# CogitatorTech/vq

Hardware: AMD Instinct MI355X
Metric: pq_encode_vectors_per_s (higher is better)
Workload: dtype f32 (bf16x3-split MFMA screen, exact f32 re-check)

## Files before the change

include/vqhip.h:

```cpp
#ifndef VQHIP_H
#define VQHIP_H

#include <stddef.h>
#include <stdint.h>

#ifdef __cplusplus
extern "C" {
#endif

#define VQHIP_VERSION_MAJOR 0
#define VQHIP_VERSION_MINOR 1

#define VQHIP_OK 0
#define VQHIP_ERR_NULL_PTR (-1)
#define VQHIP_ERR_INVALID_INPUT (-3)
#define VQHIP_ERR_NO_DEVICE (-4)
#define VQHIP_ERR_RUNTIME (-5)
#define VQHIP_ERR_UNSUPPORTED (-6)
#define VQHIP_ERR_FAILURE (-99)

#define VQHIP_SQUARED_EUCLIDEAN 0
#define VQHIP_EUCLIDEAN 1
#define VQHIP_MANHATTAN 2
#define VQHIP_COSINE 3
// ... 13 lines not shown
const char *vqhip_backend(void);
const char *vqhip_last_error(void);
int vqhip_device_count(void);
int vqhip_set_device(int device);
int vqhip_get_device(int *device);
int vqhip_set_stream(void *hip_stream);
int vqhip_synchronize(void);
int vqhip_selftest(float *bf16_32x32x16_ratio, float *bf16_16x16x32_ratio, int *bf16_engine_trusted);
int vqhip_mfma_bf16_probe(const uint16_t *a, const uint16_t *b, const float *c, uint64_t trials, float *d);
int vqhip_mfma_bf16_model(const uint16_t *a, const uint16_t *b, const float *c, uint64_t trials, float *d);
int vqhip_mfma_bf16_model_check(uint64_t trials, uint64_t seed, uint64_t *mismatches, uint64_t *first_bad_trial);
int vqhip_mfma_bf16_model_failures(uint64_t trials, uint64_t seed, uint64_t *trial_ids, uint32_t cap, uint64_t *n_failures);
int vqhip_mfma_bf16_model_case(uint64_t seed, uint64_t trial, uint16_t *a, uint16_t *b, float *c);
int vqhip_last_assign_stats(uint64_t *rechecked, int *engine);
int vqhip_last_screen_products(int *products);

int vqhip_set_profiling(int on);
int vqhip_profile_collect(uint32_t *n_calls, double *primary_ms, double *recheck_ms);
int vqhip_xfer_lane_calls(uint64_t *calls);
int vqhip_memcpy_device(void *dst, const void *src, uint64_t bytes);

int vqhip_dataset_from_host(const float *rows, uint64_t n, uint32_t d, vqhip_dataset **out);
int vqhip_dataset_from_device(const void *dev_rows, uint64_t n, uint32_t d, vqhip_dataset **out);
int vqhip_dataset_synthetic(uint64_t n, uint32_t d, uint64_t seed, uint64_t row_offset,
                            vqhip_dataset **out);
int vqhip_dataset_info(const vqhip_dataset *ds, uint64_t *n, uint32_t *d, const void **dev_rows);
int vqhip_dataset_read(const vqhip_dataset *ds, uint64_t row0, uint64_t nrows, float *out);
int vqhip_dataset_destroy(vqhip_dataset *ds);
int vqhip_synth_uniform_host(float *out, uint64_t n, uint32_t d, uint64_t seed,
                             uint64_t row_offset);
// ... 283 lines not shown
```

vq_amd/_lib.py:

```python
from __future__ import annotations

import ctypes as C
import os

import numpy as np

from . import _arena

from .errors import FfiError

_HERE = os.path.dirname(os.path.abspath(__file__))
LIB_PATH = os.environ.get("VQHIP_LIB_PATH", os.path.join(_HERE, "libvqhip.so"))

OK = 0
ERR_NULL_PTR, ERR_INVALID_INPUT, ERR_NO_DEVICE, ERR_RUNTIME, ERR_UNSUPPORTED, ERR_FAILURE = (
    -1, -3, -4, -5, -6, -99)

SQUARED_EUCLIDEAN, EUCLIDEAN, MANHATTAN, COSINE, COSINE_UNCLAMPED = 0, 1, 2, 3, 4
IVF_RESIDUAL = 1
ENGINE_AUTO, ENGINE_EXACT, ENGINE_MFMA, ENGINE_MFMA_BF16 = 0, 1, 2, 3

_u8p = C.POINTER(C.c_uint8)
_u16p = C.POINTER(C.c_uint16)
_u32p = C.POINTER(C.c_uint32)
# ... 1 lines not shown
_i32p = C.POINTER(C.c_int32)
_f32p = C.POINTER(C.c_float)
_vp = C.c_void_p
_vpp = C.POINTER(C.c_void_p)

SIGNATURES = {
    "vqhip_backend": (C.c_char_p, []),
    "vqhip_last_error": (C.c_char_p, []),
    "vqhip_device_count": (C.c_int, []),
    "vqhip_set_device": (C.c_int, [C.c_int]),
    "vqhip_get_device": (C.c_int, [C.POINTER(C.c_int)]),
    "vqhip_set_stream": (C.c_int, [_vp]),
    "vqhip_synchronize": (C.c_int, []),
    "vqhip_last_assign_stats": (C.c_int, [_u64p, C.POINTER(C.c_int)]),
    "vqhip_last_screen_products": (C.c_int, [C.POINTER(C.c_int)]),
    "vqhip_xfer_lane_calls": (C.c_int, [C.POINTER(C.c_uint64)]),
    "vqhip_set_profiling": (C.c_int, [C.c_int]),
    "vqhip_profile_collect": (C.c_int, [_u32p, C.POINTER(C.c_double), C.POINTER(C.c_double)]),
    "vqhip_memcpy_device": (C.c_int, [_vp, _vp, C.c_uint64]),
    "vqhip_code_bytes": (C.c_uint32, [C.c_uint32]),
    "vqhip_dataset_from_host": (C.c_int, [_f32p, C.c_uint64, C.c_uint32, _vpp]),
    "vqhip_dataset_from_device": (C.c_int, [_vp, C.c_uint64, C.c_uint32, _vpp]),
    "vqhip_dataset_synthetic": (C.c_int, [C.c_uint64, C.c_uint32, C.c_uint64, C.c_uint64, _vpp]),
    "vqhip_dataset_info": (C.c_int, [_vp, _u64p, _u32p, _vpp]),
    "vqhip_dataset_read": (C.c_int, [_vp, C.c_uint64, C.c_uint64, _f32p]),
    "vqhip_dataset_destroy": (C.c_int, [_vp]),
    "vqhip_synth_uniform_host": (C.c_int, [_f32p, C.c_uint64, C.c_uint32, C.c_uint64, C.c_uint64]),
    "vqhip_kmeans_create": (C.c_int, [_vp, C.c_uint32, C.c_uint32, _vpp]),
    "vqhip_kmeans_destroy": (C.c_int, [_vp]),
    "vqhip_kmeans_set_centroids": (C.c_int, [_vp, _f32p]),
# ... 1132 lines not shown
    check(load().vqhip_memcpy_device(C.c_void_p(dst), C.c_void_p(src), nbytes))


def last_assign_stats():
    r, e = C.c_uint64(), C.c_int()
    check(load().vqhip_last_assign_stats(C.byref(r), C.byref(e)))
    return int(r.value), int(e.value)


def last_screen_products() -> int:
    p = C.c_int()
    check(load().vqhip_last_screen_products(C.byref(p)))
    return int(p.value)


def param_check(rc: int) -> None:
    if rc == OK:
        return
    import re

    from .errors import InvalidParameter

    msg = last_error()
    m = re.fullmatch(r"Invalid parameter '([^']*)': (.*)", msg, flags=re.S)
    if rc == ERR_INVALID_INPUT and m:
        raise InvalidParameter(m.group(1), m.group(2))
    raise FfiError(msg or f"libvqhip status {rc}", rc)


def elementwise(fn: str, params, a, in_dtype, out_dtype, out=None) -> np.ndarray:
# ... 12 lines not shown
```

vq_amd/csrc/api.hip:

```cpp
#include <algorithm>
#include <atomic>
#include <cmath>
#include <cstdlib>
#include <cstring>
#include <limits>
#include <map>
#include <memory>
#include <condition_variable>
#include <mutex>
#include <new>
#include <thread>
#include <vector>

#include "adc_plan.hpp"
#include "kernels.hpp"

namespace vqhip {

ThreadState &tls() {
    static thread_local ThreadState st;
    return st;
}

int fail(int code, const char *fmt, ...) {
// ... 1020 lines not shown

int vqhip_mfma_bf16_model_case(uint64_t seed, uint64_t trial, uint16_t *a, uint16_t *b, float *c) {
    if (!a || !b || !c) return fail(VQHIP_ERR_NULL_PTR, "NULL argument");
    mfma_bf16_model_case(seed, trial, a, b, c);
    return VQHIP_OK;
}

int vqhip_synchronize(void) {
    VQ_TRY(require_gfx950());
    hipStream_t s;
    VQ_TRY(current_stream(&s));
    VQ_HIP(hipStreamSynchronize(s));
    return VQHIP_OK;
}

int vqhip_last_assign_stats(uint64_t *rechecked, int *engine) {
    VQ_API_BEGIN
    ThreadState &st = tls();
    if (engine) *engine = st.last_engine;
    if (rechecked) {
        *rechecked = 0;
        if (!g_last_ws) return VQHIP_OK;
        WsPin pin(g_last_ws);
        if (!pin.ws) return VQHIP_OK;
        AssignWorkspace *ws = pin.ws;
        Entry in(*pin.sync);
        if (ws->stats_pending) {
            hipStream_t s;
            VQ_TRY(in.stream(&s));
            uint64_t tot = 0;
            if (ws->last_segmented) {
                if (ws->last_n_seg > 0) {
                    VQ_HIP(hipMemcpyAsync(ws->seg_host, ws->wl_seg.p, (size_t)ws->stats_m * ws->last_n_seg * 8, hipMemcpyDeviceToHost, s));
                    VQ_HIP(hipStreamSynchronize(s));
                    for (size_t i = 0; i < (size_t)ws->stats_m * ws->last_n_seg; ++i) tot += ws->seg_host[2 * i + 1];
                }
            } else {
                VQ_HIP(hipMemcpyAsync(ws->stats_host, ws->wl_count.p, (size_t)ws->stats_m * 4, hipMemcpyDeviceToHost, s));
                VQ_HIP(hipStreamSynchronize(s));
                for (uint32_t i = 0; i < ws->stats_m; ++i) tot += ws->stats_host[i];
            }
            in.synced();
            *rechecked = tot;
        }
    }
    return VQHIP_OK;
    VQ_API_END
}

int vqhip_last_screen_products(int *products) {
    if (!products) return fail(VQHIP_ERR_NULL_PTR, "NULL argument");
    const ThreadState &st = tls();
    *products = (st.last_engine == VQHIP_ENGINE_MFMA_BF16) ? st.last_products : 0;
    return VQHIP_OK;
}

int vqhip_xfer_lane_calls(uint64_t *calls) {
    if (!calls) return fail(VQHIP_ERR_NULL_PTR, "NULL argument");
    *calls = g_xfer_lane_calls.load();
    return VQHIP_OK;
// ... 3166 lines not shown
```

vq_amd/csrc/k_exact.hip:

```cpp
#include "kernels.hpp"
#include <type_traits>

#pragma clang fp contract(off)

namespace vqhip {
namespace {

constexpr int kExactBlock = 256;

template <int METRIC, int SD, bool GENERIC>
__device__ __forceinline__ uint32_t scan_one(const float *__restrict__ xrow, uint32_t sd_rt,
                                             const float *__restrict__ cbs,
                                             const float *__restrict__ cnsq, uint32_t k) {
    const uint32_t sd = GENERIC ? sd_rt : (uint32_t)SD;
    float x[GENERIC ? 1 : SD];
    if constexpr (!GENERIC) {
#pragma unroll
        for (int t = 0; t < SD; ++t) x[t] = xrow[t];
    }
    float na = 0.0f;
    if constexpr (vq_is_cos(METRIC)) {
        float sa = -0.0f;
        if constexpr (GENERIC) {
            for (uint32_t t = 0; t < sd; ++t) {
// ... 203 lines not shown
                const float dist = acc[jj][r];
                if (j == 0) {
                    best_dist = dist;
                } else if (dist < best_dist) {
                    best_dist = dist;
                    best = j;
                }
            }
        }
        __syncthreads();
    }
    if (q == 0 && row0 + r < n) store_code(codes, (row0 + r) * m + s, best, k);
}

template <int METRIC, int SD>
__device__ __forceinline__ float exact_dist_fixed(const float (&x)[SD], const float *__restrict__ c,
                                                  float na, float nb) {
    if constexpr (METRIC == VQHIP_SQUARED_EUCLIDEAN || METRIC == VQHIP_EUCLIDEAN) {
        float acc = 0.0f;
#pragma unroll
        for (int t = 0; t < SD; ++t) {
            float diff = x[t] - c[t];
            float sq = diff * diff;
            acc = acc + sq;
        }
        return (METRIC == VQHIP_EUCLIDEAN) ? sqrtf(acc) : acc;
    } else if constexpr (METRIC == VQHIP_MANHATTAN) {
        float acc = 0.0f;
#pragma unroll
        for (int t = 0; t < SD; ++t) {
            float diff = x[t] - c[t];
            acc = acc + fabsf(diff);
        }
        return acc;
    } else {
        float dot = -0.0f;
#pragma unroll
        for (int t = 0; t < SD; ++t) {
            float p = x[t] * c[t];
            dot = dot + p;
        }
        return vq_cosine_finish(METRIC, dot, na, nb);
    }
}

template <int METRIC, int SD>
__global__ __launch_bounds__(1024) void k_recheck_wave(
    const float *__restrict__ X, uint32_t d, uint32_t m, uint32_t k,
    const float *__restrict__ cb, const float *__restrict__ cnsqrt,
    const uint32_t *__restrict__ sub_list, const uint32_t *__restrict__ wl_rows,
    const uint32_t *__restrict__ wl_count, uint64_t wl_stride, const uint32_t *__restrict__ wl_seg,
    uint32_t n_seg, uint8_t *__restrict__ codes) {
    const uint32_t s = sub_list ? sub_list[blockIdx.y] : blockIdx.y;
    const uint32_t lane = threadIdx.x & 63;
    uint32_t count, first, wave, n_waves;
    if (wl_seg) {
        const uint32_t *sg = wl_seg + ((size_t)s * n_seg + blockIdx.x) * 2;
        first = sg[0];
        count = sg[1];
        wave = threadIdx.x >> 6;
        n_waves = blockDim.x >> 6;
    } else {
        first = 0;
        count = wl_count[s];
        wave = blockIdx.x * (blockDim.x >> 6) + (threadIdx.x >> 6);
        n_waves = gridDim.x * (blockDim.x >> 6);
    }
    const float *cbs = cb + (size_t)s * k * SD;
    const float *cnsq = cnsqrt ? cnsqrt + (size_t)s * k : nullptr;
    const uint32_t NONE = 0xFFFFFFFFu;
    for (uint32_t i = wave; i < count; i += n_waves) {
        const uint64_t row = wl_rows[(size_t)s * wl_stride + first + i];
        const float *xrow = X + row * d + (size_t)s * SD;
        float x[SD];
// ... 23 lines not shown
            }
        }
#pragma unroll
        for (int off = 32; off > 0; off >>= 1) {
            const float od = __shfl_xor(bd, off);
            const uint32_t oj = (uint32_t)__shfl_xor((int)bj, off);
            const bool take = (oj != NONE) && (bj == NONE || od < bd || (od == bd && oj < bj));
            bd = take ? od : bd;
            bj = take ? oj : bj;
        }
        const bool blocked = __shfl((int)d0_nan, 0) != 0;
        if (lane == 0) store_code(codes, row * m + s, (blocked || bj == NONE) ? 0u : bj, k);
    }
}

template <int CTRL>
__device__ __forceinline__ void argmin_dpp_step(float &bd, uint32_t &bj) {
    const float od = __int_as_float(__builtin_amdgcn_update_dpp(__float_as_int(bd), __float_as_int(bd), CTRL, 0xF, 0xF, false));
    const uint32_t oj = (uint32_t)__builtin_amdgcn_update_dpp((int)bj, (int)bj, CTRL, 0xF, 0xF, false);
    const bool take = (od < bd) | ((od == bd) & (oj < bj));
    bd = take ? od : bd;
    bj = take ? oj : bj;
}
__device__ __forceinline__ void argmin_wave(float &bd, uint32_t &bj) {
    argmin_dpp_step<0xB1>(bd, bj);
    argmin_dpp_step<0x4E>(bd, bj);
    argmin_dpp_step<0x141>(bd, bj);
    argmin_dpp_step<0x140>(bd, bj);
    float rd = __int_as_float(__builtin_amdgcn_readlane(__float_as_int(bd), 0));
    uint32_t rj = (uint32_t)__builtin_amdgcn_readlane((int)bj, 0);
#pragma unroll
    for (int r = 16; r < 64; r += 16) {
        const float od = __int_as_float(__builtin_amdgcn_readlane(__float_as_int(bd), r));
        const uint32_t oj = (uint32_t)__builtin_amdgcn_readlane((int)bj, r);
        const bool take = (od < rd) | ((od == rd) & (oj < rj));
        rd = take ? od : rd;
        rj = take ? oj : rj;
    }
    bd = rd;
    bj = rj;
}

template <int METRIC, int SD, int KPL>
__global__ __launch_bounds__(256) void k_recheck_resident(
    const float *__restrict__ X, uint32_t d, uint32_t m, uint32_t k,
    const float *__restrict__ cb, const float *__restrict__ cnsqrt,
    const uint32_t *__restrict__ sub_list, const uint32_t *__restrict__ wl_rows, uint64_t wl_stride,
    const uint32_t *__restrict__ wl_seg, const uint32_t *__restrict__ wl_count, uint32_t n_seg, uint32_t parts,
    uint8_t *__restrict__ codes) {
    const uint32_t s = sub_list ? sub_list[blockIdx.y] : blockIdx.y;
    const uint32_t lane = threadIdx.x & 63;
    const uint32_t wave = __builtin_amdgcn_readfirstlane(blockIdx.x * 4 + (threadIdx.x >> 6));
    const uint32_t n_waves = gridDim.x * 4;
    const float *cbs = cb + (size_t)s * k * SD;
    const uint32_t NONE = 0xFFFFFFFFu;
    constexpr bool PK = (METRIC == VQHIP_SQUARED_EUCLIDEAN || METRIC == VQHIP_EUCLIDEAN) && (KPL % 2 == 0);
    typedef float f2 __attribute__((ext_vector_type(2)));
    float c[PK ? 1 : KPL][SD];
    f2 cp[PK ? KPL / 2 : 1][SD];
    float cn[KPL];
#pragma unroll
    for (int i = 0; i < KPL; ++i) {
        const uint32_t j = lane + 64u * i;
        const float *src = cbs + (size_t)(j < k ? j : 0u) * SD;
#pragma unroll
        for (int t = 0; t < SD; t += 4) {
            const float4 v = *reinterpret_cast<const float4 *>(src + t);
            const float e[4] = {v.x, v.y, v.z, v.w};
#pragma unroll
            for (int u = 0; u < 4; ++u) {
                if constexpr (PK) {
                    if (i % 2 == 0) cp[i / 2][t + u].x = e[u];
                    else cp[i / 2][t + u].y = e[u];
                } else {
                    c[i][t + u] = e[u];
                }
            }
        }
        cn[i] = (vq_is_cos(METRIC)) ? cnsqrt[(size_t)s * k + (j < k ? j : 0u)] : 0.0f;
    }
    const uint32_t *rows_s = wl_rows + (size_t)s * wl_stride;
    for (uint32_t unit = wave; unit < n_seg * parts; unit += n_waves) {
        const uint32_t seg = unit / parts, part = unit - seg * parts;
        const uint32_t *sg = wl_seg ? wl_seg + ((size_t)s * n_seg + seg) * 2 : nullptr;
        const uint32_t seg_first = sg ? sg[0] : 0u, seg_count = sg ? sg[1] : wl_count[s];
        const uint32_t share = (seg_count + parts - 1) / parts;
        const uint32_t lo = part * share, hi = min(seg_count, lo + share);
        for (uint32_t base = lo; base < hi; base += 64) {
            const uint32_t nb = min(64u, hi - base);
            const uint32_t my_row = rows_s[seg_first + base + min(lane, nb - 1)];
            auto fetch = [&](uint32_t e, float (&x)[SD]) {
                const uint32_t row = (uint32_t)__builtin_amdgcn_readlane((int)my_row, (int)e);
                const float *xrow = X + (size_t)row * d + (size_t)s * SD;
#pragma unroll
                for (int t = 0; t < SD; t += 4) {
                    const float4 v = *reinterpret_cast<const float4 *>(xrow + t);
                    x[t] = v.x, x[t + 1] = v.y, x[t + 2] = v.z, x[t + 3] = v.w;
                }
            };
            float xn[SD];
            fetch(0, xn);
            for (uint32_t e = 0; e < nb; ++e) {
                float x[SD];
#pragma unroll
                for (int t = 0; t < SD; ++t) x[t] = xn[t];
                if (e + 1 < nb) fetch(e + 1, xn);
                float na = 0.0f;
                if constexpr (vq_is_cos(METRIC)) {
                    float sa = -0.0f;
#pragma unroll
                    for (int t = 0; t < SD; ++t) {
                        float p = x[t] * x[t];
                        sa = sa + p;
                    }
                    na = sqrtf(sa);
                }
                float bd = __builtin_inff();
                uint32_t bj = NONE;
                bool d0_nan = false;
                auto consider = [&](int i, float dist) {
                    const uint32_t j = lane + 64u * i;
                    const bool isnan_d = dist != dist;
                    if (i == 0) d0_nan = isnan_d && (lane == 0);
                    const bool better = (j < k) & !isnan_d & ((bj == NONE) | (dist < bd));
                    bd = better ? dist : bd;
                    bj = better ? j : bj;
                };
                if constexpr (PK) {
#pragma unroll
                    for (int p = 0; p < KPL / 2; ++p) {
                        f2 acc = {0.0f, 0.0f};
#pragma unroll
                        for (int t = 0; t < SD; ++t) {
                            const f2 xx = {x[t], x[t]};
                            const f2 diff = xx - cp[p][t];
                            const f2 sq = diff * diff;
                            acc = acc + sq;
                        }
                        consider(2 * p, (METRIC == VQHIP_EUCLIDEAN) ? sqrtf(acc.x) : acc.x);
                        consider(2 * p + 1, (METRIC == VQHIP_EUCLIDEAN) ? sqrtf(acc.y) : acc.y);
                    }
                } else {
#pragma unroll
                    for (int i = 0; i < KPL; ++i) consider(i, exact_dist_fixed<METRIC, SD>(x, c[i], na, cn[i]));
                }
                argmin_wave(bd, bj);
                const bool blocked = __builtin_amdgcn_readlane((int)d0_nan, 0) != 0;
                const uint32_t row = (uint32_t)__builtin_amdgcn_readlane((int)my_row, (int)e);
                if (lane == 0) store_code(codes, (size_t)row * m + s, (blocked || bj == NONE) ? 0u : bj, k);
            }
        }
    }
}

template <int METRIC, int SD>
__global__ __launch_bounds__(1024) void k_recheck_tiled(
    const float *__restrict__ X, uint32_t d, uint32_t m, uint32_t k, const float *__restrict__ cb,
    const float *__restrict__ cnsqrt, const uint32_t *__restrict__ sub_list, const uint32_t *__restrict__ wl_rows,
    const uint32_t *__restrict__ wl_count, uint64_t wl_stride, uint8_t *__restrict__ codes) {
    constexpr uint32_t TCN = 64, PITCH = SD + 4;
    __shared__ __attribute__((aligned(16))) float ct[TCN][PITCH];
    __shared__ __attribute__((aligned(16))) float xs[16][SD];
    const uint32_t s = sub_list ? sub_list[blockIdx.y] : blockIdx.y;
    const uint32_t lane = threadIdx.x & 63, wave = threadIdx.x >> 6;
    const uint32_t count = wl_count[s];
// ... 498 lines not shown
```

vq_amd/csrc/k_screen_bf16.hip:

```cpp
#include <cstdlib>

#include "kernels.hpp"

namespace vqhip {
namespace {

typedef float f32x4 __attribute__((ext_vector_type(4)));
typedef short bf16x8 __attribute__((ext_vector_type(8)));
typedef unsigned int u32x4 __attribute__((ext_vector_type(4)));

constexpr int kWavesPerBlock = 4;
constexpr int kBlock = kWavesPerBlock * 64;
constexpr uint64_t kPipeMinSteps = 8;

__host__ __device__ constexpr int pair_a(int p) { return p == 0 ? 0 : p == 1 ? 1 : p == 2 ? 0 : p == 3 ? 2 : p == 4 ? 1 : 0; }
__host__ __device__ constexpr int pair_x(int p) { return p == 0 ? 0 : p == 1 ? 0 : p == 2 ? 1 : p == 3 ? 0 : p == 4 ? 1 : 2; }

__host__ __device__ inline void split3(float v, uint32_t (&part)[3]) {
    uint32_t b0, b1, b2;
#if defined(__HIP_DEVICE_COMPILE__)
    b0 = __float_as_uint(v) & 0xFFFF0000u;
    const float r1 = v - __uint_as_float(b0);
    b1 = __float_as_uint(r1) & 0xFFFF0000u;
    const float r2 = r1 - __uint_as_float(b1);
// ... 576 lines not shown
        sg[1] = seg_count;
    }
}

#ifndef VQ_ACC_F64
#define VQ_ACC_F64 1
#endif
#ifndef VQ_ACC_RELOAD_PAR
#define VQ_ACC_RELOAD_PAR 0
#endif
__host__ __device__ constexpr uint32_t x32p_acc_plane_bytes(int nt32) { return (uint32_t)nt32 * 32u * 8u; }
__host__ __device__ constexpr uint32_t x32p_acc_bytes_per_wave(int sd, int nt32) {
    return (uint32_t)sd * x32p_acc_plane_bytes(nt32) + 64u + ((uint32_t)nt32 * 32u + 64u) * 4u;
}

template <int SD, int NT32, bool ACC = false, int NPR = 6, int PVW = 0>
__global__ __launch_bounds__(kBlock, x32_two_waves(SD, NT32, NPR) ? 2 : 1) void k_assign_screen_bf16_x32p(
    const float *__restrict__ X, uint64_t n, uint32_t d, uint32_t m, const uint32_t *__restrict__ prepA32,
    const float *__restrict__ prepCn, uint32_t cn_stride, const float *__restrict__ meta,
    const uint32_t *__restrict__ sub_list, uint32_t n_sub, uint8_t *__restrict__ codes, uint32_t *__restrict__ wl_rows,
    uint32_t *__restrict__ wl_seg, uint32_t n_seg, uint64_t wl_stride, int cosine, uint32_t k_real,
    const float *__restrict__ cen, const uint8_t *__restrict__ gate_active, const uint32_t *__restrict__ gate_halt,
    uint8_t *__restrict__ codes_t, uint64_t codes_t_pitch, float *__restrict__ acc_sums, uint32_t *__restrict__ acc_counts,
    uint32_t sdr) {
    static_assert(NT32 == 8 && (SD == 8 || SD == 16), "pipelined screen: 8 tiles, sub_dim 8 or 16");
    static_assert(NPR == 6 || (NPR == 3 && SD == 16 && !ACC), "three products: sub_dim 16, encode form");
    static_assert(PVW == 0 || NPR == 3, "padded rows: three-product form only");
    constexpr int DPH = SD / 2;
    constexpr int NMF = (NPR * DPH + 7) / 8;
    static_assert(NPR * DPH == 8 * NMF, "every MFMA carries one term pair (sub_dim 16) or two (sub_dim 8), no padding slots");
    constexpr bool kTwo = x32_two_waves(SD, NT32, NPR);
    const bool halted = gate_halt && *gate_halt;
    const uint32_t lane = threadIdx.x & 63;
    const uint32_t h = lane >> 5, p = lane & 31;
    const uint32_t wave = __builtin_amdgcn_readfirstlane(threadIdx.x >> 6);
    const uint32_t gw = blockIdx.x * kWavesPerBlock + wave;
    const uint32_t n_chunks = n_seg;
    if (gw >= n_chunks * n_sub) return;
    const uint32_t vv = gw % n_sub;
    const uint32_t s = sub_list[vv];
// ... 59 lines not shown
            uint32_t *pc = acc_counts + ((size_t)chunk * n_sub + vv) * k_real;
            for (uint32_t e = lane; e < k_real; e += 64) pc[e] = cnts[e];
        }
    };
#endif
    if (st0 >= st1) {
        write_partial();
        if (lane == 0) seg_hdr[0] = 0u, seg_hdr[1] = 0u;
        return;
    }
    const uint32_t nst = st1 - st0;
    const uint32_t seg_first = st0 * 32;
    uint32_t seg_count = 0;

    __shared__ __attribute__((aligned(16))) float lds_cn[kWavesPerBlock][NT32 * 32];
    bf16x8 a[NT32][NMF];
    {
        const uint32_t *base = prepA32 + (size_t)s * NT32 * NMF * 4 * 64 + lane;
#pragma unroll
        for (int i = 0; i < NT32; ++i)
#pragma unroll
            for (int f = 0; f < NMF; ++f) {
                u32x4 v;
#pragma unroll
                for (int w = 0; w < 4; ++w) v[w] = base[((i * NMF + f) * 4 + w) * 64];
                a[i][f] = __builtin_bit_cast(bf16x8, v);
            }
        const float *pc = prepCn + (size_t)s * cn_stride;
        for (uint32_t e = lane; e < NT32 * 32; e += 64) {
            float v = (e < cn_stride) ? pc[e] : 3.0e38f;
// ... 354 lines not shown
            bool proven = (gap > T) && (fabsf(t_m1) <= 3.0e38f) && (T <= 3.0e38f);
            if (cosine) proven = proven && (t_m1 < -T) && (xnorm > 4e-10f);
            t_proven = proven;
        } else {
            const bool valid = in_loop ? !no_step : (tst < st1);
            const uint32_t row = (in_loop && !valid ? st0 : tst) * 32 + p;
            const uint32_t rowc = row < n32 ? row : n32 - 1;
            if (in_loop || valid) code_base[(uint64_t)rowc * code_stride] = (uint8_t)t_j;
            const bool writer = (h == 0) && (row < n32) && valid;
            const bool recheck = writer && !t_proven;
            const unsigned long long mask = __ballot(recheck);
            if (mask != 0ull) {
                if (recheck) {
                    const uint32_t rank = (uint32_t)__popcll(mask & ((1ull << lane) - 1ull));
                    wl_rows[(size_t)s * wl_stride + seg_first + seg_count + rank] = (uint32_t)row;
                }
                seg_count += (uint32_t)__popcll(mask);
            }
            acc_ticket(t_proven && valid && (row < n32));
        }
    };

    float held_m1 = 0.0f, held_m2 = 0.0f, held_xs = 0.0f;
    uint32_t held_j = 0;
    auto tail_hold = [&]() { held_m1 = t_m1, held_m2 = t_m2, held_j = t_j, held_xs = xsT; };
    auto tail_pair_piece = [&](int k, uint32_t S, bool first) {
        if (k == 1) {
            const auto r1 = __builtin_amdgcn_permlane32_swap(__float_as_uint(held_m1), __float_as_uint(t_m1), false, false);
            const auto r2 = __builtin_amdgcn_permlane32_swap(__float_as_uint(held_m2), __float_as_uint(t_m2), false, false);
            const auto rj = __builtin_amdgcn_permlane32_swap(held_j, t_j, false, false);
// ... 11 lines not shown
            const bool valid = (h != 0) || !first;
            const uint32_t row = (S - 1 + h) * 32 + p;
            uint32_t srow = row, sj = t_j;
            if (first) {
                sj = __builtin_amdgcn_permlane32_swap(t_j, t_j, false, false)[1];
                srow = S * 32 + p;
            }
            const uint32_t rowc = srow < n32 ? srow : n32 - 1;
            code_base[(uint64_t)rowc * code_stride] = (uint8_t)sj;
            const bool recheck = valid && (row < n32) && !t_proven;
            const unsigned long long mask = __ballot(recheck);
            if (mask != 0ull) {
                if (recheck) {
                    const uint32_t rank = (uint32_t)__popcll(mask & ((1ull << lane) - 1ull));
                    wl_rows[(size_t)s * wl_stride + seg_first + seg_count + rank] = (uint32_t)row;
                }
                seg_count += (uint32_t)__popcll(mask);
            }
            acc_update_begin(valid && (row < n32) && t_proven);
        }
    };

    load_x(st0 * 32 + p, 0);
    if (kDeep == 2) load_x((st0 + 1) * 32 + p, 1);
#pragma unroll
    for (int k = 0; k < kSplitPieces; ++k) split_piece(k, 0, st0 + kDeep);
    xsM = xsN;
#pragma unroll
    for (int c = 0; c < 2; ++c) q1[0][c] = q2[0][c] = q1[1][c] = q2[1][c] = pinf;
    if (0 >= kCnV) init_acc(acc[0], 0);
// ... 85 lines not shown
            }
            xsT = xsM;
            xsM = xsN;
        }
      }
    }
    {
        const uint32_t last = st0 + ((nst + 1) & ~1u) - 1;
        acc_reload(last);
#pragma unroll
        for (int k = 0; k < 4; ++k) tail_piece(k, 1, last, false);
        acc_issue();
        acc_commit();
        write_partial();
    }
    if (lane == 0) seg_hdr[0] = seg_first, seg_hdr[1] = seg_count;
}

template <int G>
__global__ __launch_bounds__(256) void k_merge_partials_x32(const uint4 *__restrict__ part, uint64_t n, uint32_t m,
                                                            uint32_t sd, const uint32_t *__restrict__ sub_list,
                                                            const float *__restrict__ cen, const float *__restrict__ meta,
                                                            int cosine, uint8_t *__restrict__ codes,
                                                            uint32_t *__restrict__ wl_rows, uint32_t *__restrict__ wl_count,
                                                            uint64_t wl_stride, uint32_t k, uint32_t groups_rt) {
    const uint32_t groups = (G > 0) ? (uint32_t)G : groups_rt;
    const uint32_t s = sub_list[blockIdx.y];
    const float *cs = cen + (size_t)s * (sd + 4);
    float cmax = cs[sd], tcoef = cs[sd + 1];
    if (cosine) {
        const float nmf = (float)((6 * (sd / 2) + 7) / 8);
// ... 267 lines not shown
        dyn_lds = (size_t)kWavesPerBlock * NT32 * 32 * (x32_acc_copies(SD, NT32) * SD + 1) * 4;
        static PerDeviceOnce attr_set;
        if (attr_set.needed()) {
            VQ_HIP(hipFuncSetAttribute(reinterpret_cast<const void *>(k_assign_screen_bf16_x32<SD, NT32, G, PVW, ACC>),
                                       hipFuncAttributeMaxDynamicSharedMemorySize, 160 * 1024 - 8 * 1024));
            attr_set.done();
        }
    }
    bool piped = false;
    if constexpr (G == 1 && SD == 16 && NT32 == 8 && !ACC && PVW != 4) {
        if (use3) {
            piped = true;
            hipLaunchKernelGGL((k_assign_screen_bf16_x32p<SD, NT32, false, 3, PVW>), dim3(blocks), dim3(kBlock), 0, stream, a.X, a.n, a.d,
                               cb.m, cb.prepA32_3, cb.cn32, NT32 * 32, cb.meta, a.sub_list, a.n_sub, a.codes, a.wl_rows, a.wl_seg,
                               n_chunks, a.wl_stride, 0, cb.k, cb.cen, a.gate_active, a.gate_halt, a.codes_t, a.codes_t_pitch,
                               nullptr, nullptr, cb.sd);
        }
    }
    if constexpr (G == 1 && PVW == 0 && NT32 == 8 && (SD == 16 || SD == 8)) {
        const uint64_t steps_per_chunk = (n_steps + n_chunks - 1) / n_chunks;
        if (!piped && pipe_on && steps_per_chunk >= kPipeMinSteps && a.n < 0xFFFFFFC0ull) {
            piped = true;
            if constexpr (ACC) {
                static PerDeviceOnce attr_set_p;
                if (attr_set_p.needed()) {
                    VQ_HIP(hipFuncSetAttribute(reinterpret_cast<const void *>(k_assign_screen_bf16_x32p<SD, NT32, ACC>),
                                               hipFuncAttributeMaxDynamicSharedMemorySize, 160 * 1024 - 8 * 1024));
                    attr_set_p.done();
                }
            }
            const size_t dyn_lds_p = (ACC && VQ_ACC_F64) ? (size_t)kWavesPerBlock * x32p_acc_bytes_per_wave(SD, NT32) : dyn_lds;
            hipLaunchKernelGGL((k_assign_screen_bf16_x32p<SD, NT32, ACC>), dim3(blocks), dim3(kBlock), dyn_lds_p, stream, a.X, a.n, a.d,
                               cb.m, cb.prepA32, cb.cn32, NT32 * 32, cb.meta, a.sub_list, a.n_sub, a.codes, a.wl_rows, a.wl_seg,
                               n_chunks, a.wl_stride, a.metric == VQHIP_COSINE ? 1 : 0, cb.k, cb.cen, a.gate_active,
                               a.gate_halt, a.codes_t, a.codes_t_pitch, ACC ? a.acc_sums : nullptr, ACC ? a.acc_counts : nullptr,
                               (uint32_t)SD);
        }
    }
    if (!piped)
        hipLaunchKernelGGL((k_assign_screen_bf16_x32<SD, NT32, G, PVW, ACC>), dim3(blocks), dim3(kBlock), dyn_lds, stream, a.X, a.n, a.d,
                           cb.m, cb.prepA32, cb.cn32, NT32 * groups * 32, cb.meta, a.sub_list, a.n_sub, a.codes, a.wl_rows,
                           a.wl_seg, n_chunks, a.wl_stride, a.metric == VQHIP_COSINE ? 1 : 0, cb.k, cb.cen,
                           reinterpret_cast<uint4 *>(a.part), groups, cb.sd, ACC ? a.acc_sums : nullptr, ACC ? a.acc_counts : nullptr,
                           a.gate_active, a.gate_halt, (G == 1) ? a.codes_t : nullptr, a.codes_t_pitch);
    VQ_LAUNCH_CHECK("k_assign_screen_bf16_x32");
    if (G == 1 && a.codes_t) {
        hipLaunchKernelGGL(k_codes_transpose, dim3((uint32_t)((a.n + 255) / 256)), dim3(256), (size_t)256 * codes_transpose_pitch(cb.m) + cb.m, stream,
                           a.codes_t, a.codes_t_pitch, a.codes, a.n, cb.m, a.sub_list, a.n_sub, a.gate_active, a.gate_halt);
        VQ_LAUNCH_CHECK("k_codes_transpose");
    }
    if (G != 1) {
// ... 210 lines not shown
```

vq_amd/csrc/kernels.hpp:

```cpp
#pragma once

#include <mutex>
#include <vector>

#include "common.hpp"

namespace vqhip {

__host__ __device__ __forceinline__ uint32_t code_bytes(uint32_t k) { return k <= 256u ? 1u : 2u; }
__device__ __forceinline__ uint32_t load_code(const uint8_t *codes, size_t i, uint32_t k) {
    return k <= 256u ? (uint32_t)codes[i] : (uint32_t)reinterpret_cast<const uint16_t *>(codes)[i];
}
__device__ __forceinline__ void store_code(uint8_t *codes, size_t i, uint32_t j, uint32_t k) {
    if (k <= 256u) codes[i] = (uint8_t)j;
    else reinterpret_cast<uint16_t *>(codes)[i] = (uint16_t)j;
}
constexpr uint32_t kMaxCentroids = 65536;
constexpr uint32_t kX32MaxGroups = 16;

struct CodebookView {
    uint32_t m = 0, k = 0, sd = 0;
    const float *cb = nullptr;
    uint32_t nt = 0, ks = 0;
    const float *prepA = nullptr;
    const float *prepCn = nullptr;
    const float *meta = nullptr;
    const float *cnsqrt = nullptr;
    const uint32_t *prepA32 = nullptr;
    const uint32_t *prepA32_3 = nullptr;
    const float *cen = nullptr;
    const float *cn32 = nullptr;
};

// ... 341 lines not shown
```

Before: 3.447 billion.

## Fuse exact f32 recheck into the bf16 screen kernel for small segments

In the three-product encode screen kernel, rows flagged for exact recheck are also staged in LDS. When a wave's segment has at most the cap of flagged rows, the kernel loads the exact centroids into registers and resolves those rows in place. It then marks the segment header as settled, so the later recheck kernels skip it. This is meant to cut the separate recheck pass's work and its scattered re-reads of rows, at the cost of extra registers, LDS and a serial tail inside the screen kernel, which may reduce its occupancy.

```diff
diff --git a/include/vqhip.h b/include/vqhip.h
--- a/include/vqhip.h
+++ b/include/vqhip.h
@@ -51,6 +51,7 @@
 int vqhip_mfma_bf16_model_case(uint64_t seed, uint64_t trial, uint16_t *a, uint16_t *b, float *c);
 int vqhip_last_assign_stats(uint64_t *rechecked, int *engine);
 int vqhip_last_screen_products(int *products);
+int vqhip_last_recheck_split(uint64_t *in_kernel, uint64_t *published);
 
 int vqhip_set_profiling(int on);
 int vqhip_profile_collect(uint32_t *n_calls, double *primary_ms, double *recheck_ms);
diff --git a/vq_amd/_lib.py b/vq_amd/_lib.py
--- a/vq_amd/_lib.py
+++ b/vq_amd/_lib.py
@@ -39,6 +39,7 @@
     "vqhip_synchronize": (C.c_int, []),
     "vqhip_last_assign_stats": (C.c_int, [_u64p, C.POINTER(C.c_int)]),
     "vqhip_last_screen_products": (C.c_int, [C.POINTER(C.c_int)]),
+    "vqhip_last_recheck_split": (C.c_int, [C.POINTER(C.c_uint64), C.POINTER(C.c_uint64)]),
     "vqhip_xfer_lane_calls": (C.c_int, [C.POINTER(C.c_uint64)]),
     "vqhip_set_profiling": (C.c_int, [C.c_int]),
     "vqhip_profile_collect": (C.c_int, [_u32p, C.POINTER(C.c_double), C.POINTER(C.c_double)]),
@@ -1201,6 +1202,12 @@
     return int(p.value)
 
 
+def last_recheck_split():
+    a, b = C.c_uint64(), C.c_uint64()
+    check(load().vqhip_last_recheck_split(C.byref(a), C.byref(b)))
+    return int(a.value), int(b.value)
+
+
 def param_check(rc: int) -> None:
     if rc == OK:
         return
diff --git a/vq_amd/csrc/api.hip b/vq_amd/csrc/api.hip
--- a/vq_amd/csrc/api.hip
+++ b/vq_amd/csrc/api.hip
@@ -1058,12 +1058,10 @@
     return VQHIP_OK;
 }
 
-int vqhip_last_assign_stats(uint64_t *rechecked, int *engine) {
-    VQ_API_BEGIN
-    ThreadState &st = tls();
-    if (engine) *engine = st.last_engine;
-    if (rechecked) {
+static int fetch_recheck_counts(uint64_t *rechecked, uint64_t *in_kernel) {
+    {
         *rechecked = 0;
+        *in_kernel = 0;
         if (!g_last_ws) return VQHIP_OK;
         WsPin pin(g_last_ws);
         if (!pin.ws) return VQHIP_OK;
@@ -1072,12 +1070,15 @@
         if (ws->stats_pending) {
             hipStream_t s;
             VQ_TRY(in.stream(&s));
-            uint64_t tot = 0;
+            uint64_t tot = 0, fused = 0;
             if (ws->last_segmented) {
                 if (ws->last_n_seg > 0) {
                     VQ_HIP(hipMemcpyAsync(ws->seg_host, ws->wl_seg.p, (size_t)ws->stats_m * ws->last_n_seg * 8, hipMemcpyDeviceToHost, s));
                     VQ_HIP(hipStreamSynchronize(s));
-                    for (size_t i = 0; i < (size_t)ws->stats_m * ws->last_n_seg; ++i) tot += ws->seg_host[2 * i + 1];
+                    for (size_t i = 0; i < (size_t)ws->stats_m * ws->last_n_seg; ++i) {
+                        tot += ws->seg_host[2 * i + 1];
+                        if (ws->seg_host[2 * i] & kSegSettled) fused += ws->seg_host[2 * i + 1];
+                    }
                 }
             } else {
                 VQ_HIP(hipMemcpyAsync(ws->stats_host, ws->wl_count.p, (size_t)ws->stats_m * 4, hipMemcpyDeviceToHost, s));
@@ -1086,8 +1087,29 @@
             }
             in.synced();
             *rechecked = tot;
-        }
-    }
+            *in_kernel = fused;
+        }
+    }
+    return VQHIP_OK;
+}
+
+int vqhip_last_assign_stats(uint64_t *rechecked, int *engine) {
+    VQ_API_BEGIN
+    if (engine) *engine = tls().last_engine;
+    if (rechecked) {
+        uint64_t fused;
+        VQ_TRY(fetch_recheck_counts(rechecked, &fused));
+    }
+    return VQHIP_OK;
+    VQ_API_END
+}
+
+int vqhip_last_recheck_split(uint64_t *in_kernel, uint64_t *published) {
+    VQ_API_BEGIN
+    if (!in_kernel || !published) return fail(VQHIP_ERR_NULL_PTR, "NULL argument");
+    uint64_t tot;
+    VQ_TRY(fetch_recheck_counts(&tot, in_kernel));
+    *published = tot - *in_kernel;
     return VQHIP_OK;
     VQ_API_END
 }
diff --git a/vq_amd/csrc/k_exact.hip b/vq_amd/csrc/k_exact.hip
--- a/vq_amd/csrc/k_exact.hip
+++ b/vq_amd/csrc/k_exact.hip
@@ -1,4 +1,5 @@
 #include "kernels.hpp"
+#include "recheck_body.hpp"
 #include <type_traits>
 
 #pragma clang fp contract(off)
@@ -241,37 +242,6 @@
 }
 
 template <int METRIC, int SD>
-__device__ __forceinline__ float exact_dist_fixed(const float (&x)[SD], const float *__restrict__ c,
-                                                  float na, float nb) {
-    if constexpr (METRIC == VQHIP_SQUARED_EUCLIDEAN || METRIC == VQHIP_EUCLIDEAN) {
-        float acc = 0.0f;
-#pragma unroll
-        for (int t = 0; t < SD; ++t) {
-            float diff = x[t] - c[t];
-            float sq = diff * diff;
-            acc = acc + sq;
-        }
-        return (METRIC == VQHIP_EUCLIDEAN) ? sqrtf(acc) : acc;
-    } else if constexpr (METRIC == VQHIP_MANHATTAN) {
-        float acc = 0.0f;
-#pragma unroll
-        for (int t = 0; t < SD; ++t) {
-            float diff = x[t] - c[t];
-            acc = acc + fabsf(diff);
-        }
-        return acc;
-    } else {
-        float dot = -0.0f;
-#pragma unroll
-        for (int t = 0; t < SD; ++t) {
-            float p = x[t] * c[t];
-            dot = dot + p;
-        }
-        return vq_cosine_finish(METRIC, dot, na, nb);
-    }
-}
-
-template <int METRIC, int SD>
 __global__ __launch_bounds__(1024) void k_recheck_wave(
     const float *__restrict__ X, uint32_t d, uint32_t m, uint32_t k,
     const float *__restrict__ cb, const float *__restrict__ cnsqrt,
@@ -283,8 +253,8 @@
     uint32_t count, first, wave, n_waves;
     if (wl_seg) {
         const uint32_t *sg = wl_seg + ((size_t)s * n_seg + blockIdx.x) * 2;
-        first = sg[0];
-        count = sg[1];
+        first = sg[0] & ~kSegSettled;
+        count = (sg[0] & kSegSettled) ? 0u : sg[1];
         wave = threadIdx.x >> 6;
         n_waves = blockDim.x >> 6;
     } else {
@@ -338,33 +308,6 @@
     }
 }
 
-template <int CTRL>
-__device__ __forceinline__ void argmin_dpp_step(float &bd, uint32_t &bj) {
-    const float od = __int_as_float(__builtin_amdgcn_update_dpp(__float_as_int(bd), __float_as_int(bd), CTRL, 0xF, 0xF, false));
-    const uint32_t oj = (uint32_t)__builtin_amdgcn_update_dpp((int)bj, (int)bj, CTRL, 0xF, 0xF, false);
-    const bool take = (od < bd) | ((od == bd) & (oj < bj));
-    bd = take ? od : bd;
-    bj = take ? oj : bj;
-}
-__device__ __forceinline__ void argmin_wave(float &bd, uint32_t &bj) {
-    argmin_dpp_step<0xB1>(bd, bj);
-    argmin_dpp_step<0x4E>(bd, bj);
-    argmin_dpp_step<0x141>(bd, bj);
-    argmin_dpp_step<0x140>(bd, bj);
-    float rd = __int_as_float(__builtin_amdgcn_readlane(__float_as_int(bd), 0));
-    uint32_t rj = (uint32_t)__builtin_amdgcn_readlane((int)bj, 0);
-#pragma unroll
-    for (int r = 16; r < 64; r += 16) {
-        const float od = __int_as_float(__builtin_amdgcn_readlane(__float_as_int(bd), r));
-        const uint32_t oj = (uint32_t)__builtin_amdgcn_readlane((int)bj, r);
-        const bool take = (od < rd) | ((od == rd) & (oj < rj));
-        rd = take ? od : rd;
-        rj = take ? oj : rj;
-    }
-    bd = rd;
-    bj = rj;
-}
-
 template <int METRIC, int SD, int KPL>
 __global__ __launch_bounds__(256) void k_recheck_resident(
     const float *__restrict__ X, uint32_t d, uint32_t m, uint32_t k,
@@ -376,103 +319,34 @@
     const uint32_t lane = threadIdx.x & 63;
     const uint32_t wave = __builtin_amdgcn_readfirstlane(blockIdx.x * 4 + (threadIdx.x >> 6));
     const uint32_t n_waves = gridDim.x * 4;
-    const float *cbs = cb + (size_t)s * k * SD;
-    const uint32_t NONE = 0xFFFFFFFFu;
-    constexpr bool PK = (METRIC == VQHIP_SQUARED_EUCLIDEAN || METRIC == VQHIP_EUCLIDEAN) && (KPL % 2 == 0);
-    typedef float f2 __attribute__((ext_vector_type(2)));
-    float c[PK ? 1 : KPL][SD];
-    f2 cp[PK ? KPL / 2 : 1][SD];
-    float cn[KPL];
-#pragma unroll
-    for (int i = 0; i < KPL; ++i) {
-        const uint32_t j = lane + 64u * i;
-        const float *src = cbs + (size_t)(j < k ? j : 0u) * SD;
-#pragma unroll
-        for (int t = 0; t < SD; t += 4) {
-            const float4 v = *reinterpret_cast<const float4 *>(src + t);
-            const float e[4] = {v.x, v.y, v.z, v.w};
-#pragma unroll
-            for (int u = 0; u < 4; ++u) {
-                if constexpr (PK) {
-                    if (i % 2 == 0) cp[i / 2][t + u].x = e[u];
-                    else cp[i / 2][t + u].y = e[u];
-                } else {
-                    c[i][t + u] = e[u];
-                }
-            }
-        }
-        cn[i] = (vq_is_cos(METRIC)) ? cnsqrt[(size_t)s * k + (j < k ? j : 0u)] : 0.0f;
-    }
     const uint32_t *rows_s = wl_rows + (size_t)s * wl_stride;
-    for (uint32_t unit = wave; unit < n_seg * parts; unit += n_waves) {
+    auto unit_share = [&](uint32_t unit, uint32_t &seg_first, uint32_t &lo, uint32_t &hi) {
         const uint32_t seg = unit / parts, part = unit - seg * parts;
         const uint32_t *sg = wl_seg ? wl_seg + ((size_t)s * n_seg + seg) * 2 : nullptr;
-        const uint32_t seg_first = sg ? sg[0] : 0u, seg_count = sg ? sg[1] : wl_count[s];
+        const uint32_t h0 = sg ? sg[0] : 0u;
+        const uint32_t seg_count = (h0 & kSegSettled) ? 0u : sg ? sg[1] : wl_count[s];
+        seg_first = h0 & ~kSegSettled;
         const uint32_t share = (seg_count + parts - 1) / parts;
-        const uint32_t lo = part * share, hi = min(seg_count, lo + share);
+        lo = part * share, hi = min(seg_count, lo + share);
+        return lo < hi;
+    };
+    {
+        bool work = false;
+        uint32_t f, lo, hi;
+        for (uint32_t unit = wave; unit < n_seg * parts && !work; unit += n_waves) work = unit_share(unit, f, lo, hi);
+        if (!work) return;
+    }
+    ResidentCentroids<METRIC, SD, KPL> cen;
+    cen.load(cb + (size_t)s * k * SD, vq_is_cos(METRIC) ? cnsqrt + (size_t)s * k : nullptr, lane, k);
+    const float *xs = X + (size_t)s * SD;
+    for (uint32_t unit = wave; unit < n_seg * parts; unit += n_waves) {
+        uint32_t seg_first, lo, hi;
+        if (!unit_share(unit, seg_first, lo, hi)) continue;
         for (uint32_t base = lo; base < hi; base += 64) {
             const uint32_t nb = min(64u, hi - base);
             const uint32_t my_row = rows_s[seg_first + base + min(lane, nb - 1)];
-            auto fetch = [&](uint32_t e, float (&x)[SD]) {
-                const uint32_t row = (uint32_t)__builtin_amdgcn_readlane((int)my_row, (int)e);
-                const float *xrow = X + (size_t)row * d + (size_t)s * SD;
-#pragma unroll
-                for (int t = 0; t < SD; t += 4) {
-                    const float4 v = *reinterpret_cast<const float4 *>(xrow + t);
-                    x[t] = v.x, x[t + 1] = v.y, x[t + 2] = v.z, x[t + 3] = v.w;
-                }
-            };
-            float xn[SD];
-            fetch(0, xn);
-            for (uint32_t e = 0; e < nb; ++e) {
-                float x[SD];
-#pragma unroll
-                for (int t = 0; t < SD; ++t) x[t] = xn[t];
-                if (e + 1 < nb) fetch(e + 1, xn);
-                float na = 0.0f;
-                if constexpr (vq_is_cos(METRIC)) {
-                    float sa = -0.0f;
-#pragma unroll
-                    for (int t = 0; t < SD; ++t) {
-                        float p = x[t] * x[t];
-                        sa = sa + p;
-                    }
-                    na = sqrtf(sa);
-                }
-                float bd = __builtin_inff();
-                uint32_t bj = NONE;
-                bool d0_nan = false;
-                auto consider = [&](int i, float dist) {
-                    const uint32_t j = lane + 64u * i;
-                    const bool isnan_d = dist != dist;
-                    if (i == 0) d0_nan = isnan_d && (lane == 0);
-                    const bool better = (j < k) & !isnan_d & ((bj == NONE) | (dist < bd));
-                    bd = better ? dist : bd;
-                    bj = better ? j : bj;
-                };
-                if constexpr (PK) {
-#pragma unroll
-                    for (int p = 0; p < KPL / 2; ++p) {
-                        f2 acc = {0.0f, 0.0f};
-#pragma unroll
-                        for (int t = 0; t < SD; ++t) {
-                            const f2 xx = {x[t], x[t]};
-                            const f2 diff = xx - cp[p][t];
-                            const f2 sq = diff * diff;
-                            acc = acc + sq;
-                        }
-                        consider(2 * p, (METRIC == VQHIP_EUCLIDEAN) ? sqrtf(acc.x) : acc.x);
-                        consider(2 * p + 1, (METRIC == VQHIP_EUCLIDEAN) ? sqrtf(acc.y) : acc.y);
-                    }
-                } else {
-#pragma unroll
-                    for (int i = 0; i < KPL; ++i) consider(i, exact_dist_fixed<METRIC, SD>(x, c[i], na, cn[i]));
-                }
-                argmin_wave(bd, bj);
-                const bool blocked = __builtin_amdgcn_readlane((int)d0_nan, 0) != 0;
-                const uint32_t row = (uint32_t)__builtin_amdgcn_readlane((int)my_row, (int)e);
-                if (lane == 0) store_code(codes, (size_t)row * m + s, (blocked || bj == NONE) ? 0u : bj, k);
-            }
+            recheck_batch(cen, xs, d, my_row, nb, lane, k, METRIC == VQHIP_EUCLIDEAN,
+                          [&](uint32_t row, uint32_t code) { store_code(codes, (size_t)row * m + s, code, k); });
         }
     }
 }
diff --git a/vq_amd/csrc/k_screen_bf16.hip b/vq_amd/csrc/k_screen_bf16.hip
--- a/vq_amd/csrc/k_screen_bf16.hip
+++ b/vq_amd/csrc/k_screen_bf16.hip
@@ -1,6 +1,7 @@
 #include <cstdlib>
 
 #include "kernels.hpp"
+#include "recheck_body.hpp"
 
 namespace vqhip {
 namespace {
@@ -614,6 +615,11 @@
     return (uint32_t)sd * x32p_acc_plane_bytes(nt32) + 64u + ((uint32_t)nt32 * 32u + 64u) * 4u;
 }
 
+#ifndef VQ_FUSE_CAP
+#define VQ_FUSE_CAP 32
+#endif
+constexpr uint32_t kFuseCap = VQ_FUSE_CAP;
+static_assert(kFuseCap >= 1 && kFuseCap <= 64, "one recheck_batch of at most 64 entries");
 template <int SD, int NT32, bool ACC = false, int NPR = 6, int PVW = 0>
 __global__ __launch_bounds__(kBlock, x32_two_waves(SD, NT32, NPR) ? 2 : 1) void k_assign_screen_bf16_x32p(
     const float *__restrict__ X, uint64_t n, uint32_t d, uint32_t m, const uint32_t *__restrict__ prepA32,
@@ -622,8 +628,9 @@
     uint32_t *__restrict__ wl_seg, uint32_t n_seg, uint64_t wl_stride, int cosine, uint32_t k_real,
     const float *__restrict__ cen, const uint8_t *__restrict__ gate_active, const uint32_t *__restrict__ gate_halt,
     uint8_t *__restrict__ codes_t, uint64_t codes_t_pitch, float *__restrict__ acc_sums, uint32_t *__restrict__ acc_counts,
-    uint32_t sdr) {
+    uint32_t sdr, const float *__restrict__ cb_exact, int euclid) {
     static_assert(NT32 == 8 && (SD == 8 || SD == 16), "pipelined screen: 8 tiles, sub_dim 8 or 16");
+    constexpr bool kFuse = !ACC && NPR == 3 && PVW == 0;
     static_assert(NPR == 6 || (NPR == 3 && SD == 16 && !ACC), "three products: sub_dim 16, encode form");
     static_assert(PVW == 0 || NPR == 3, "padded rows: three-product form only");
     constexpr int DPH = SD / 2;
@@ -713,6 +720,11 @@
     uint32_t seg_count = 0;
 
     __shared__ __attribute__((aligned(16))) float lds_cn[kWavesPerBlock][NT32 * 32];
+    uint32_t *fuse_rows = nullptr;
+    if constexpr (kFuse) {
+        __shared__ uint32_t lds_rows[kWavesPerBlock][kFuseCap];
+        fuse_rows = lds_rows[wave];
+    }
     bf16x8 a[NT32][NMF];
     {
         const uint32_t *base = prepA32 + (size_t)s * NT32 * NMF * 4 * 64 + lane;
@@ -1097,6 +1109,9 @@
                 if (recheck) {
                     const uint32_t rank = (uint32_t)__popcll(mask & ((1ull << lane) - 1ull));
                     wl_rows[(size_t)s * wl_stride + seg_first + seg_count + rank] = (uint32_t)row;
+                    if constexpr (kFuse) {
+                        if (seg_count + rank < kFuseCap) fuse_rows[seg_count + rank] = (uint32_t)row;
+                    }
                 }
                 seg_count += (uint32_t)__popcll(mask);
             }
@@ -1138,6 +1153,9 @@
                 if (recheck) {
                     const uint32_t rank = (uint32_t)__popcll(mask & ((1ull << lane) - 1ull));
                     wl_rows[(size_t)s * wl_stride + seg_first + seg_count + rank] = (uint32_t)row;
+                    if constexpr (kFuse) {
+                        if (seg_count + rank < kFuseCap) fuse_rows[seg_count + rank] = (uint32_t)row;
+                    }
                 }
                 seg_count += (uint32_t)__popcll(mask);
             }
@@ -1253,7 +1271,19 @@
         acc_commit();
         write_partial();
     }
-    if (lane == 0) seg_hdr[0] = seg_first, seg_hdr[1] = seg_count;
+    uint32_t settled = 0u;
+    if constexpr (kFuse) {
+        if (seg_count != 0u && seg_count <= kFuseCap) {
+            ResidentCentroids<VQHIP_SQUARED_EUCLIDEAN, SD, NT32 / 2> cen;
+            cen.load(cb_exact + (size_t)s * k_real * SD, nullptr, lane, k_real);
+            const uint32_t my_row = fuse_rows[lane < seg_count ? lane : seg_count - 1u];
+            asm volatile("s_waitcnt vmcnt(0)" ::: "memory");
+            recheck_batch(cen, X + sub0, d, my_row, seg_count, lane, k_real, euclid != 0,
+                          [&](uint32_t row, uint32_t code) { code_base[(uint64_t)row * code_stride] = (uint8_t)code; });
+            settled = kSegSettled;
+        }
+    }
+    if (lane == 0) seg_hdr[0] = seg_first | settled, seg_hdr[1] = seg_count;
 }
 
 template <int G>
@@ -1551,7 +1581,7 @@
             hipLaunchKernelGGL((k_assign_screen_bf16_x32p<SD, NT32, false, 3, PVW>), dim3(blocks), dim3(kBlock), 0, stream, a.X, a.n, a.d,
                                cb.m, cb.prepA32_3, cb.cn32, NT32 * 32, cb.meta, a.sub_list, a.n_sub, a.codes, a.wl_rows, a.wl_seg,
                                n_chunks, a.wl_stride, 0, cb.k, cb.cen, a.gate_active, a.gate_halt, a.codes_t, a.codes_t_pitch,
-                               nullptr, nullptr, cb.sd);
+                               nullptr, nullptr, cb.sd, cb.cb, a.metric == VQHIP_EUCLIDEAN ? 1 : 0);
         }
     }
     if constexpr (G == 1 && PVW == 0 && NT32 == 8 && (SD == 16 || SD == 8)) {
@@ -1571,7 +1601,7 @@
                                cb.m, cb.prepA32, cb.cn32, NT32 * 32, cb.meta, a.sub_list, a.n_sub, a.codes, a.wl_rows, a.wl_seg,
                                n_chunks, a.wl_stride, a.metric == VQHIP_COSINE ? 1 : 0, cb.k, cb.cen, a.gate_active,
                                a.gate_halt, a.codes_t, a.codes_t_pitch, ACC ? a.acc_sums : nullptr, ACC ? a.acc_counts : nullptr,
-                               (uint32_t)SD);
+                               (uint32_t)SD, nullptr, 0);
         }
     }
     if (!piped)
diff --git a/vq_amd/csrc/kernels.hpp b/vq_amd/csrc/kernels.hpp
--- a/vq_amd/csrc/kernels.hpp
+++ b/vq_amd/csrc/kernels.hpp
@@ -17,6 +17,7 @@
 }
 constexpr uint32_t kMaxCentroids = 65536;
 constexpr uint32_t kX32MaxGroups = 16;
+constexpr uint32_t kSegSettled = 1u;
 
 struct CodebookView {
     uint32_t m = 0, k = 0, sd = 0;
diff --git a/vq_amd/csrc/recheck_body.hpp b/vq_amd/csrc/recheck_body.hpp
--- /dev/null
+++ b/vq_amd/csrc/recheck_body.hpp
@@ -0,0 +1,169 @@
+#pragma once
+
+#include "kernels.hpp"
+
+namespace vqhip {
+
+template <int METRIC, int SD>
+__device__ __forceinline__ float exact_dist_fixed(const float (&x)[SD], const float *__restrict__ c,
+                                                  float na, float nb) {
+#pragma clang fp contract(off)
+    if constexpr (METRIC == VQHIP_SQUARED_EUCLIDEAN || METRIC == VQHIP_EUCLIDEAN) {
+        float acc = 0.0f;
+#pragma unroll
+        for (int t = 0; t < SD; ++t) {
+            float diff = x[t] - c[t];
+            float sq = diff * diff;
+            acc = acc + sq;
+        }
+        return (METRIC == VQHIP_EUCLIDEAN) ? sqrtf(acc) : acc;
+    } else if constexpr (METRIC == VQHIP_MANHATTAN) {
+        float acc = 0.0f;
+#pragma unroll
+        for (int t = 0; t < SD; ++t) {
+            float diff = x[t] - c[t];
+            acc = acc + fabsf(diff);
+        }
+        return acc;
+    } else {
+        float dot = -0.0f;
+#pragma unroll
+        for (int t = 0; t < SD; ++t) {
+            float p = x[t] * c[t];
+            dot = dot + p;
+        }
+        return vq_cosine_finish(METRIC, dot, na, nb);
+    }
+}
+
+template <int CTRL>
+__device__ __forceinline__ void argmin_dpp_step(float &bd, uint32_t &bj) {
+    const float od = __int_as_float(__builtin_amdgcn_update_dpp(__float_as_int(bd), __float_as_int(bd), CTRL, 0xF, 0xF, false));
+    const uint32_t oj = (uint32_t)__builtin_amdgcn_update_dpp((int)bj, (int)bj, CTRL, 0xF, 0xF, false);
+    const bool take = (od < bd) | ((od == bd) & (oj < bj));
+    bd = take ? od : bd;
+    bj = take ? oj : bj;
+}
+__device__ __forceinline__ void argmin_wave(float &bd, uint32_t &bj) {
+    argmin_dpp_step<0xB1>(bd, bj);
+    argmin_dpp_step<0x4E>(bd, bj);
+    argmin_dpp_step<0x141>(bd, bj);
+    argmin_dpp_step<0x140>(bd, bj);
+    float rd = __int_as_float(__builtin_amdgcn_readlane(__float_as_int(bd), 0));
+    uint32_t rj = (uint32_t)__builtin_amdgcn_readlane((int)bj, 0);
+#pragma unroll
+    for (int r = 16; r < 64; r += 16) {
+        const float od = __int_as_float(__builtin_amdgcn_readlane(__float_as_int(bd), r));
+        const uint32_t oj = (uint32_t)__builtin_amdgcn_readlane((int)bj, r);
+        const bool take = (od < rd) | ((od == rd) & (oj < rj));
+        rd = take ? od : rd;
+        rj = take ? oj : rj;
+    }
+    bd = rd;
+    bj = rj;
+}
+
+template <int METRIC, int SD, int KPL>
+struct ResidentCentroids {
+    static constexpr bool PK = (METRIC == VQHIP_SQUARED_EUCLIDEAN || METRIC == VQHIP_EUCLIDEAN) && (KPL % 2 == 0);
+    typedef float f2 __attribute__((ext_vector_type(2)));
+    float c[PK ? 1 : KPL][SD];
+    f2 cp[PK ? KPL / 2 : 1][SD];
+    float cn[KPL];
+
+    __device__ __forceinline__ void load(const float *__restrict__ cbs, const float *__restrict__ cnsq_s, uint32_t lane, uint32_t k) {
+#pragma unroll
+        for (int i = 0; i < KPL; ++i) {
+            const uint32_t j = lane + 64u * i;
+            const float *src = cbs + (size_t)(j < k ? j : 0u) * SD;
+#pragma unroll
+            for (int t = 0; t < SD; t += 4) {
+                const float4 v = *reinterpret_cast<const float4 *>(src + t);
+                const float e[4] = {v.x, v.y, v.z, v.w};
+#pragma unroll
+                for (int u = 0; u < 4; ++u) {
+                    if constexpr (PK) {
+                        if (i % 2 == 0) cp[i / 2][t + u].x = e[u];
+                        else cp[i / 2][t + u].y = e[u];
+                    } else {
+                        c[i][t + u] = e[u];
+                    }
+                }
+            }
+            cn[i] = (vq_is_cos(METRIC)) ? cnsq_s[j < k ? j : 0u] : 0.0f;
+        }
+    }
+};
+
+template <int METRIC, int SD, int KPL, class Store>
+__device__ __forceinline__ void recheck_batch(const ResidentCentroids<METRIC, SD, KPL> &cen, const float *__restrict__ xs,
+                                              uint32_t d, uint32_t my_row, uint32_t nb, uint32_t lane, uint32_t k, bool root,
+                                              Store store) {
+#pragma clang fp contract(off)
+    using RC = ResidentCentroids<METRIC, SD, KPL>;
+    typedef typename RC::f2 f2;
+    const uint32_t NONE = 0xFFFFFFFFu;
+    auto fetch = [&](uint32_t e, float (&x)[SD]) {
+        const uint32_t row = (uint32_t)__builtin_amdgcn_readlane((int)my_row, (int)e);
+        const float *xrow = xs + (size_t)row * d;
+#pragma unroll
+        for (int t = 0; t < SD; t += 4) {
+            const float4 v = *reinterpret_cast<const float4 *>(xrow + t);
+            x[t] = v.x, x[t + 1] = v.y, x[t + 2] = v.z, x[t + 3] = v.w;
+        }
+    };
+    float xn[SD];
+    fetch(0, xn);
+    for (uint32_t e = 0; e < nb; ++e) {
+        float x[SD];
+#pragma unroll
+        for (int t = 0; t < SD; ++t) x[t] = xn[t];
+        if (e + 1 < nb) fetch(e + 1, xn);
+        float na = 0.0f;
+        if constexpr (vq_is_cos(METRIC)) {
+            float sa = -0.0f;
+#pragma unroll
+            for (int t = 0; t < SD; ++t) {
+                float p = x[t] * x[t];
+                sa = sa + p;
+            }
+            na = sqrtf(sa);
+        }
+        float bd = __builtin_inff();
+        uint32_t bj = NONE;
+        bool d0_nan = false;
+        auto consider = [&](int i, float dist) {
+            const uint32_t j = lane + 64u * i;
+            const bool isnan_d = dist != dist;
+            if (i == 0) d0_nan = isnan_d && (lane == 0);
+            const bool better = (j < k) & !isnan_d & ((bj == NONE) | (dist < bd));
+            bd = better ? dist : bd;
+            bj = better ? j : bj;
+        };
+        if constexpr (RC::PK) {
+#pragma unroll
+            for (int p = 0; p < KPL / 2; ++p) {
+                f2 acc = {0.0f, 0.0f};
+#pragma unroll
+                for (int t = 0; t < SD; ++t) {
+                    const f2 xx = {x[t], x[t]};
+                    const f2 diff = xx - cen.cp[p][t];
+                    const f2 sq = diff * diff;
+                    acc = acc + sq;
+                }
+                if (root) acc.x = sqrtf(acc.x), acc.y = sqrtf(acc.y);
+                consider(2 * p, acc.x);
+                consider(2 * p + 1, acc.y);
+            }
+        } else {
+#pragma unroll
+            for (int i = 0; i < KPL; ++i) consider(i, exact_dist_fixed<METRIC, SD>(x, cen.c[i], na, cen.cn[i]));
+        }
+        argmin_wave(bd, bj);
+        const bool blocked = __builtin_amdgcn_readlane((int)d0_nan, 0) != 0;
+        const uint32_t row = (uint32_t)__builtin_amdgcn_readlane((int)my_row, (int)e);
+        if (lane == 0) store(row, (blocked || bj == NONE) ? 0u : bj);
+    }
+}
+
+}
```

New measurement: 3.422 billion. No clear change (-0.7%).
